# nygenome/lancet

Hardware: AMD Instinct MI355X
Metric: assembled windows/sec (whole node), 600bp windows, self-tuning k, synthetic T/N (higher is better)
Workload: dtype u64; 1 GPU; chr22-scan proxy: 32768 windows/GPU x 600 bp, stride 100, 30x tumor / 30x normal, 2x150 bp, k=11..101, active-region-off; windows_per_gpu=32768, reads_per_gpu=5895305, records_rank0_contig=22477, slots_in_flight=4080, batches_in_flight=2, windows_first_graph_in_lds=32768, graphs_built_ahead=2147, graphs_taken_from_pool=2037, windows_rerun_worst_case_tier=0

## Files before the change

lancet_amd/csrc/build_lds_impl.h:

```cpp
namespace BL_NS {

#if BL_OFFBITS > 16
typedef uint32_t bl_occ_t;
typedef uint32_t bl_off_t;
#else
typedef uint16_t bl_occ_t;
typedef uint16_t bl_off_t;
#endif
static constexpr uint32_t BL_OFFMASK = (1u << BL_OFFBITS) - 1u;
#if BL_WIDE
typedef uint32_t bl_on_t;
static constexpr uint32_t ON_ID = 0xFFFFFu, ON_OVL = 0x40000000u, ON_ORI = 0x80000000u, ON_ORISH = 31u;
#else
typedef uint16_t bl_on_t;
static constexpr uint32_t ON_ID = 0x1FFFu, ON_OVL = 0x4000u, ON_ORI = 0x8000u, ON_ORISH = 15u;
#endif
static_assert(BL_NCAP <= ON_ID + 1u && BL_SLOTS <= ON_ID + 1u && BL_NCAP < 65536u, "node ids / slots in a per-occurrence word");
static constexpr uint32_t LDS_BASES = BL_BASES, LDS_READS = BL_RMAX;
static_assert(BL_BASES < (1u << BL_OFFBITS) && BL_BASES / 16 + 4 < 65536, "offsets of the packed reads");

struct BlShared {
  uint32_t bases[BL_BASES / 16 + 4];
  uint32_t goodm[BL_BASES / 32 + 4];
  uint16_t rdo[BL_RMAX + 4];
// ... 5 lines not shown
  uint8_t prole[BL_RMAX + 4];
#if !BL_WIDE
  uint16_t idoff[BL_NCAP];
#endif
  alignas(8) uint16_t cidx[BL_NCAP];
  uint16_t t2c[BL_TCAP];
  alignas(16) uint32_t big[BL_BIG / 4];
  uint32_t wsum[BL_WG / 64 + 1];
  uint32_t scan_total;
  int w, R, reflen, K, hasN, mapped;
  uint32_t O, N, T, ncand, nsurv, nbw, ngw;
  uint32_t totalreadbp, n_kmers;
  int repE, repM;
  int why;
  uint32_t npairs, flagged, edges_total, refn;
  uint32_t g0, g1;
  uint32_t hint;
  uint32_t ndup;
  unsigned long long t_last, ph_acc[16]; int ph_cur;
};

struct BlScratch {
  LC_GLOBAL bl_on_t *occn;
  LC_GLOBAL uint32_t *idoff;
  LC_GLOBAL unsigned long long *tcc;
  LC_GLOBAL uint32_t *tfl;
  LC_GLOBAL uint32_t *c_id;
  LC_GLOBAL uint32_t *c_ti;
  LC_GLOBAL uint32_t *c_minqv;
  LC_GLOBAL uint32_t *s_ci;
  LC_GLOBAL uint32_t *s_edges;
  LC_GLOBAL bl_off_t *dupo;
  LC_GLOBAL uint32_t *ord;
  LC_GLOBAL uint32_t *pq;
};
static constexpr uint32_t BL_PQCAP = 16384u;
static constexpr uint32_t SCRATCH_BYTES = (((uint32_t)sizeof(bl_on_t) * BL_BASES + 64u + (BL_WIDE ? 4u * BL_NCAP + 64u : 64u) + 8u * BL_TCAP + 4u * BL_TCAP + 12u * PB_CCAP + 4u * PB_SCAP + 36u * PB_SCAP + (uint32_t)sizeof(bl_off_t) * BL_DUPCAP + 16u * PB_CMAX + 4u * 16384u + 768u) + 255u) & ~255u;
static constexpr int WG = BL_WG;
DEV void bl_scratch_carve(BlScratch *s, LC_GLOBAL uint8_t *base) {
  size_t o = 0;
  auto take = [&](size_t bytes) { LC_GLOBAL uint8_t *p = base + o; o = (o + bytes + 63) & ~(size_t)63; return p; };
  s->occn = (LC_GLOBAL bl_on_t *)take(sizeof(bl_on_t) * BL_BASES + 64u);
  s->idoff = (LC_GLOBAL uint32_t *)take(BL_WIDE ? 4u * BL_NCAP : 4u);
  s->tcc = (LC_GLOBAL unsigned long long *)take(8u * BL_TCAP);
  s->tfl = (LC_GLOBAL uint32_t *)take(4u * BL_TCAP);
  s->c_id = (LC_GLOBAL uint32_t *)take(4u * PB_CCAP);
  s->c_ti = (LC_GLOBAL uint32_t *)take(4u * PB_CCAP);
  s->c_minqv = (LC_GLOBAL uint32_t *)take(4u * PB_CCAP);
  s->s_ci = (LC_GLOBAL uint32_t *)take(4u * PB_SCAP);
  s->s_edges = (LC_GLOBAL uint32_t *)take(36u * PB_SCAP);
  s->dupo = (LC_GLOBAL bl_off_t *)take(sizeof(bl_off_t) * BL_DUPCAP);
  s->ord = (LC_GLOBAL uint32_t *)take(16u * PB_CMAX);
  s->pq = (LC_GLOBAL uint32_t *)take(4u * BL_PQCAP);
}

static_assert(sizeof(BlShared) <= BL_LDS_LIMIT, "LDS of the build kernel: 2 x 80 KB (512 lanes) or 1 x 160 KB (1024 lanes) per CU");
typedef LC_LDS BlShared BL_S;
#ifndef LANCET_WAVE_EMU
static __shared__ BlShared bl_shared;
template <class P> DEV unsigned long long dev_atomic_add64(P p, unsigned long long v) { return __hip_atomic_fetch_add(p, v, __ATOMIC_RELAXED, __HIP_MEMORY_SCOPE_WORKGROUP); }
template <class P> DEV unsigned long long dev_atomic_or64(P p, unsigned long long v) { return __hip_atomic_fetch_or(p, v, __ATOMIC_RELAXED, __HIP_MEMORY_SCOPE_WORKGROUP); }
#else
DEV unsigned long long dev_atomic_add64(unsigned long long *p, unsigned long long v) { unsigned long long o = *p; *p = o + v; return o; }
DEV unsigned long long dev_atomic_or64(unsigned long long *p, unsigned long long v) { unsigned long long o = *p; *p = o | v; return o; }
#endif

#define bl_bcast(p) wg_bcastu(p)

template <class T> DEV void bl_scan_t(LC_LDS T *a, int n, BL_S &S) {
  WG_SYNC();
#ifndef LANCET_WAVE_EMU
  const int t = (int)threadIdx.x, chunk = (n + BL_WG - 1) / BL_WG;
  int lo = t * chunk, hi = lo + chunk; if (lo > n) lo = n; if (hi > n) hi = n;
  uint32_t s = 0;
  for (int i = lo; i < hi; ++i) s += a[i];
  uint32_t inc = s; const int lane = t & 63;
  for (int d = 1; d < 64; d <<= 1) { const uint32_t x = (uint32_t)__shfl_up((int)inc, d, 64); if (lane >= d) inc += x; }
  if (lane == 63) S.wsum[t >> 6] = inc;
  __syncthreads();
  uint32_t woff = 0;
  for (int i = 0; i < (t >> 6); ++i) woff += S.wsum[i];
  uint32_t run = woff + inc - s;
  for (int i = lo; i < hi; ++i) { const uint32_t x = a[i]; a[i] = (T)run; run += x; }
  if (t == BL_WG - 1) S.scan_total = run;
  __syncthreads();
// ... 231 lines not shown
template <class F> DEV void bl_for_occ(BL_S &S, LC_GLOBAL const bl_on_t *occn, F body) {
  bl_for_chunk(S, occn, [&](const BlChunk &ch, const BlOccW &w) {
    for (int j = 0; j < ch.nv; ++j) body(ch.r, ch.p0 + j, ch.boff0 + (uint32_t)j, bl_occw_get(w, j));
  });
}
DEV void bl_chunk_bases(const LC_LDS uint32_t *bases, int c, unsigned long long &lo, unsigned long long &hi) {
  const uint32_t wd = (uint32_t)c >> 1;
  lo = (unsigned long long)bases[wd] | ((unsigned long long)bases[wd + 1] << 32); hi = (unsigned long long)bases[wd + 2];
  if (c & 1) { lo = (lo >> 16) | (hi << 48); hi >>= 16; }
}


#ifdef LANCET_PROF_A
#define BLPA(S, id) BLP(S, id)
#else
#define BLPA(S, id) ((void)0)
#endif
#ifdef LANCET_PROF_ORDER
#define BLPO(S, id) BLP(S, id)
#else
#define BLPO(S, id) ((void)0)
#endif
#define BLC_TO(e) ((uint32_t)(e) & 0x3FFu)
#define BLC_DIR(e) (((uint32_t)(e) >> 10) & 3u)
#define BLC_MAKE(to, dir) ((uint16_t)((to) | ((dir) << 10)))
DEVNI void bl_compress_first(LC_GLOBAL const lancet_params *P, LC_GLOBAL const EngineCaps *C, BL_S &S, BlScratch &X, LC_GLOBAL uint8_t *area, const int K_,
                             const uint32_t N_, const uint32_t nsurv_, const uint32_t ncand_, const int reflen_, const uint32_t ht_bc_, const uint32_t refmask_) {
  P = lc_sgpr(P); C = lc_sgpr(C); area = lc_sgpr(area);
  const uint32_t N = lc_sgpr(N_), nsurv = lc_sgpr(nsurv_), ncand = lc_sgpr(ncand_), ht_bc = lc_sgpr(ht_bc_); const int reflen = lc_sgpr(reflen_);
  const int K = lc_sgpr(K_); const uint32_t refmask = lc_sgpr(refmask_);
  LC_GLOBAL const PreLayout &PL = C->pl;
  LC_GLOBAL PreCmp *CH = (LC_GLOBAL PreCmp *)(area + PRE_OFF_CHDR);
  LC_GLOBAL const uint32_t *occ_ref = (LC_GLOBAL const uint32_t *)(area + PRE_OFF_OCCREF);
  LC_GLOBAL const unsigned long long *nhash = (LC_GLOBAL const unsigned long long *)(area + PRE_OFF_NHASH);
  LC_GLOBAL const unsigned long long *skey = (LC_GLOBAL const unsigned long long *)(area + PRE_OFF_SKEY);
  LC_GLOBAL const uint32_t *sidv = (LC_GLOBAL const uint32_t *)(area + PRE_OFF_SID);
  LC_GLOBAL NodeGr *pgr = (LC_GLOBAL NodeGr *)(area + PRE_OFF_PGR);
  LC_GLOBAL const uint16_t *qv = (LC_GLOBAL const uint16_t *)(area + PRE_OFF_QV);
  LC_GLOBAL uint32_t *clive = (LC_GLOBAL uint32_t *)(area + PRE_OFF_CLIVE);
  LC_GLOBAL uint32_t *cseq = (LC_GLOBAL uint32_t *)(area + PRE_OFF_CSEQ);
  const uint32_t Pn = nsurv + 2u, SRC = nsurv, SNK = nsurv + 1u;
  const bool recov = lc_sgpr((int)P->kmer_recovery) != 0;
  LC_LDS uint8_t *arena = (LC_LDS uint8_t *)&S.bases[0];
  LC_LDS uint16_t *pos2si = (LC_LDS uint16_t *)(arena + 70304);
  LC_LDS uint16_t *E = (LC_LDS uint16_t *)arena;
  LC_LDS uint8_t *NE = arena + 13376;
  LC_LDS uint8_t *FL = arena + 14272;
  LC_LDS uint16_t *SI2POS = (LC_LDS uint16_t *)(arena + 15168);
  LC_LDS uint32_t *LNK = (LC_LDS uint32_t *)(arena + 16896);
  LC_LDS unsigned long long *PT = (LC_LDS unsigned long long *)(arena + 23616);
  LC_LDS uint32_t *HS = (LC_LDS uint32_t *)(arena + 36992);
  LC_LDS uint32_t *AL = (LC_LDS uint32_t *)(arena + 40384);
  LC_LDS uint16_t *HEADOF = (LC_LDS uint16_t *)(arena + 43776);
  LC_LDS uint8_t *INFO = arena + 45504;
  LC_LDS uint16_t *HX = (LC_LDS uint16_t *)(arena + 46400);
  LC_LDS uint16_t *HL = (LC_LDS uint16_t *)(arena + 48128);
  LC_LDS uint32_t *HACC = (LC_LDS uint32_t *)(arena + 48640);
  LC_LDS uint16_t *NEWE = (LC_LDS uint16_t *)(arena + 52736);
  LC_LDS uint16_t *NPOS = (LC_LDS uint16_t *)(arena + 59392);
  LC_LDS unsigned long long *ORD = (LC_LDS unsigned long long *)(arena + 59392);
  LC_LDS unsigned long long *TCC = (LC_LDS unsigned long long *)(arena + 74400);
  LC_LDS uint16_t *CI = (LC_LDS uint16_t *)(arena + 67584);
  static_assert(74400 + 8 * PB_CMAX <= offsetof(BlShared, big) + BL_BIG && 8 * PB_CMAX <= 2 * 4096 && 67584 + 2 * PB_CMAX <= 70304, "compress arena (2)");
  static_assert(13376 >= (PB_CMAX + 2) * 16 && 14272 - 13376 >= PB_CMAX + 2 && 16896 - 15168 >= 2 * PB_CMAX && 23616 - 16896 >= 8 * (PB_CMAX + 2) &&
                36992 - 23616 >= 16 * (PB_CMAX + 2) && 40384 - 36992 >= 4 * (PB_CMAX + 3) && 45504 - 43776 >= 2 * (PB_CMAX + 2) && 48128 - 46400 >= 2 * (PB_CMAX + 2) &&
                52736 - 48640 >= 16 * PB_CHEADS && 59392 - 52736 >= 26 * PB_CHEADS && 59392 + 2 * 4096 <= 70304, "compress arena");
  WG_LANE0 { CH->done = 0; S.why = 0; S.flagged = 0; S.g0 = 0x7FFFFFFFu; S.g1 = 0; S.ndup = 0; S.wsum[0] = 0; S.wsum[1] = 0; }
// ... 686 lines not shown
        const uint32_t id = pre[wd >> 1] + ((wd & 1u) ? (uint32_t)dev_popc(bm[wd - 1u]) : 0u) + (uint32_t)dev_popc(bm[wd] & ((1u << (off & 31u)) - 1u));
        tab[i] = id;
#if BL_WIDE
        X.idoff[id] = off;
#else
        S.idoff[id] = (uint16_t)off;
#endif
      }
    }
    WG_SYNC();
  }
  const uint32_t N = bl_bcast(&S.N);
  BLP(S, 6);
  if (C->debug_stop == 106u) { WG_LANE0 { H->why = 99; } return; }
  bl_for_chunk(S, X.occn, [&](const BlChunk &ch, const BlOccW &w) {
    uint32_t old[8];
    BL_UNROLL for (int j = 0; j < 8; ++j) {
      const bool act = j < ch.nv;
      const uint32_t e = bl_occw_get(w, j);
      old[j] = dev_atomic_add(&tab[act ? (e & (nslots - 1)) : 0u], act ? (1u << 16) : 0u);
    }
    BlOccW o = {};
    BL_UNROLL for (int j = 0; j < 8; ++j) {
      if (BL_BASES > 65535u && j < ch.nv && (old[j] >> 16) >= 0xFFFEu) S.why = BLW_SIZE;
      bl_occw_set(o, j, j < ch.nv ? ((old[j] & 0xFFFFu) | (bl_occw_get(w, j) & ON_ORI)) : 0u);
    }
    bl_occw_store(X.occn, ch.boff0, o);
  });
  WG_SYNC();
  if (BL_BASES > 65535u) { if (bl_bcast(&S.why)) { WG_LANE0 { H->why = (uint32_t)S.why; } return; } }
  BLP(S, 7);
  if (C->debug_stop == 107u) { WG_LANE0 { H->why = 99; } return; }
  {
    LC_GLOBAL unsigned long long *nhash = (LC_GLOBAL unsigned long long *)(area + PRE_OFF_NHASH);
    LC_GLOBAL uint8_t *surv = (LC_GLOBAL uint8_t *)(area + PRE_OFF_SURV);
    WG_FULL_BEGIN(n, act, N)
      unsigned long long h;
#if BL_KW > 1
      if (NW > 1) {
        BlKm v, ck, alt; bool f; bl_kmer_x(S.bases, bl_idoff(S, X, (uint32_t)n), NW, K, v); bl_canon_x(v, NW, K, ck, alt, &f);
        h = bl_std_hash_km(ck, NW, K);
      } else
#endif
      { bool f; const unsigned long long ck = bl_canon(bl_kmer(S.bases, bl_idoff(S, X, (uint32_t)n), kmask), K, kmask, &f);
        h = std_hash_bytes([&](int j) -> int { return bl_acgt((int)((ck >> (2 * (K - 1 - j))) & 3ULL)); }, K); }
      if (act) { nhash[n] = h; surv[n] = 0; }
    WG_FULL_END
  }
  const double avgcov = ((double)S.totalreadbp) / ((double)reflen);
  int tmin = 1;
  while ((tmin <= P->low_cov_threshold) || ((double)tmin <= (P->min_cov_ratio * avgcov))) ++tmin;
  const uint32_t tthr = tmin < 2 ? (uint32_t)tmin : 2u;
  WG_FOR(i, nslots) { const uint32_t e = tab[i]; if (e != BL_EMPTY) S.cidx[e & 0xFFFFu] = (uint16_t)(e >> 16); }
  WG_SYNC();
  {
    const uint32_t nd = S.ndup < BL_DUPCAP ? S.ndup : BL_DUPCAP;
    const uint32_t cthr = (uint32_t)(avgcov / 4.0) > 4u ? (uint32_t)(avgcov / 4.0) : 4u;
    WG_FOR(i, nd) { if ((uint32_t)S.cidx[X.occn[X.dupo[i]] & ON_ID] < cthr) X.dupo[i] = (bl_off_t)~(bl_off_t)0; }
  }
  {
    LC_LDS uint32_t *fl = S.big;
    WG_FOR(n, N + 1) { fl[n] = (n < (int)N && S.cidx[n] >= tthr) ? 1u : 0u; }
    bl_scan32(fl, (int)N + 1, S);
    WG_LANE0 { S.T = S.scan_total; if (S.scan_total > BL_TCAP) S.why = BLW_TRACKED; }
    if (bl_bcast(&S.why)) { WG_LANE0 { H->why = (uint32_t)S.why; } return; }
    WG_FOR(n, N) { S.cidx[n] = (fl[n + 1] != fl[n]) ? (uint16_t)fl[n] : (uint16_t)0xFFFFu; }
    WG_SYNC();
// ... 563 lines not shown
      }
      WG_SYNC();
    }
  }
  BLP(S, 15);
  BL_TAIL_PRIO_SET(BL_TAIL_PRIO);
  WG_LANE0 { H->have_order = 0; }
  const bool wide_tab = BL_WIDE != 0 && N > 4096u;
  if ((N <= 4096u || (wide_tab && N <= BL_NCAP)) && nsurv > 0) {
    LC_LDS uint8_t *arena = (LC_LDS uint8_t *)&S.bases[0];
    LC_LDS uint32_t *first = (LC_LDS uint32_t *)arena;
    LC_LDS uint32_t *tmp = first + 5120;
    LC_LDS uint16_t *Qa = (LC_LDS uint16_t *)(tmp + 4104), *Qb = Qa + 4096, *bkt = Qb + 4096, *out = bkt + 4096;
    LC_LDS unsigned long long *nh = (LC_LDS unsigned long long *)(out + 4096);
    LC_LDS uint32_t *nx = (LC_LDS uint32_t *)(nh + 32), *bk = nx + 32;
    LC_LDS uint16_t *pos2si = (LC_LDS uint16_t *)(bk + 64);
    LC_LDS uint32_t *heads = (LC_LDS uint32_t *)(pos2si + PB_SCAP);
    static_assert(5120 * 4 + 4104 * 4 + 4 * 4096 * 2 + 32 * 8 + 32 * 4 + 64 * 4 + PB_SCAP * 2 + 128 * 4 <= offsetof(BlShared, big) + BL_BIG, "order arena");
    LC_LDS uint32_t *tmpP = tmp, *numP = first; LC_LDS uint16_t *nposP = (LC_LDS uint16_t *)first, *adjP = Qa;
#if BL_WIDE
    LC_LDS uint16_t *first16 = (LC_LDS uint16_t *)arena, *tmp16 = first16 + 20768, *bktw = nullptr;
    static_assert(BL_NCAP <= 14336 && BL_NCAP < 16384, "positions / run sizes in 16 bits, bucket counts up to 20 753");
    if (wide_tab) {
      Qa = tmp16 + 14352; Qb = Qa + 14336; bktw = Qb + 14336;
      nh = (LC_LDS unsigned long long *)(bktw + 14336); nx = (LC_LDS uint32_t *)(nh + 32); bk = nx + 32; pos2si = (LC_LDS uint16_t *)(bk + 64);
      tmpP = (LC_LDS uint32_t *)arena;
      numP = tmpP + 14352;
      nposP = bktw;
      adjP = (LC_LDS uint16_t *)(tmpP + 4104);
    }
    static_assert(2 * (20768 + 14352 + 3 * 14336) + 32 * 8 + 32 * 4 + 64 * 4 + PB_SCAP * 2 <= offsetof(BlShared, big) + BL_BIG && 4 * (14352 + PB_SCAP + 1) <= 2 * (20768 + 14352) &&
                  4 * 4104 + 2 * 8 * PB_SCAP <= 4 * 14337, "order arena of the large tables");
#endif
    LC_GLOBAL const unsigned long long *nhash = (LC_GLOBAL const unsigned long long *)(area + PRE_OFF_NHASH);
    const uint32_t SEQ = 13u;
    const uint32_t n0 = N < SEQ ? N : SEQ;
    WG_SYNC();
    WG_FOR(i, n0) { nh[i] = nhash[i]; }
    WG_LANE0 {
      uint32_t bc = 1, next_resize = 0, elt = 0, head = LC_NIL;
      bk[0] = LC_NIL;
      for (uint32_t n = 0; n < n0; ++n) {
        if (elt + 1 > next_resize) {
          unsigned long long mn = elt + 1;
          if (next_resize == 0 && mn < 11) mn = 11;
          if (mn >= bc) {
            unsigned long long want = mn + 1; if (want < 2ULL * bc) want = 2ULL * bc;
            const uint32_t nb = ht_next_prime((uint32_t)want);
            next_resize = nb;
            for (uint32_t i = 0; i < nb; ++i) bk[i] = LC_NIL;
            uint32_t pp = head; head = LC_NIL; uint32_t bbegin = 0;
            while (pp != LC_NIL) {
              const uint32_t nxt = nx[pp], b = ht_mod(nh[pp], nb);
              if (bk[b] == LC_NIL) { nx[pp] = head; head = pp; bk[b] = LC_BB; if (nx[pp] != LC_NIL) bk[bbegin] = pp; bbegin = b; }
              else { const uint32_t prev = bk[b]; if (prev == LC_BB) { nx[pp] = head; head = pp; } else { nx[pp] = nx[prev]; nx[prev] = pp; } }
              pp = nxt;
            }
            bc = nb;
          } else next_resize = bc;
        }
        const uint32_t b = ht_mod(nh[n], bc), prev = bk[b];
        if (prev != LC_NIL) { if (prev == LC_BB) { nx[n] = head; head = n; } else { nx[n] = nx[prev]; nx[prev] = n; } }
        else { nx[n] = head; head = n; if (nx[n] != LC_NIL) bk[ht_mod(nh[nx[n]], bc)] = n; bk[b] = LC_BB; }
        ++elt;
      }
      uint32_t m = 0;
      for (uint32_t pp = head; pp != LC_NIL; pp = nx[pp]) Qa[m++] = (uint16_t)pp;
// ... 136 lines not shown
        while (true) {
          a = uf_find(a); b = uf_find(b);
          if (a == b) break;
          const uint32_t hi = a > b ? a : b, lo = a > b ? b : a;
          if (dev_atomic_cas32(&parent[hi], hi, lo) == hi) break;
        }
      }
    }
    WG_SYNC();
    WG_FOR(u, nsurv) { const uint32_t r = uf_find((uint32_t)u); dev_atomic_min(&parent[u], r); }
    WG_SYNC();
#endif
    WG_FOR(u, nsurv) { if (touch[u] & 1u) dev_atomic_or(&touch[parent[u]], 2u); }
    WG_SYNC();
    LC_LDS uint32_t *num = numP;
    WG_FOR(u, nsurv + 1) { num[u] = (u < (int)nsurv && parent[u] == (uint32_t)u) ? 1u : 0u; }
    bl_scan32(num, (int)nsurv + 1, S);
    WG_LANE0 { S.nbw = S.scan_total; S.ngw = 0; S.flagged = 0; }
    WG_SYNC();
    WG_FOR(u, nsurv) { if (parent[u] == (uint32_t)u && (touch[u] & 2u)) { dev_atomic_add((LC_LDS uint32_t *)&S.ngw, 1u); if (num[u] < 32u) dev_atomic_or((LC_LDS uint32_t *)&S.flagged, 1u << num[u]); } }
    LC_GLOBAL NodeGr *pgr2 = (LC_GLOBAL NodeGr *)(area + PRE_OFF_PGR);
    WG_FOR(u, nsurv) { pgr2[pos2si[u]].comp = (int)(num[parent[u]] + 1u); }
    WG_LANE0 { H->have_order = 1; H->ht_bc = S.g0; H->ht_next_resize = S.g1; H->numcomp = S.nbw; H->refcomp = S.ngw; }
    WG_SYNC();
    BLPA(S, 15); BLPO(S, 15);
    {
      WG_SYNC();
      const uint32_t hbc = lc_sgpr((uint32_t)S.g0), hnr = lc_sgpr((uint32_t)S.g1), ncomp = lc_sgpr((uint32_t)S.nbw), refmask = lc_sgpr((uint32_t)S.flagged);
      WG_SYNC();
      if ((!rep || cmp_later) && (ncomp == 1u || (!rep && ncomp <= 32u)) && nsurv <= PB_CMAX && nsurv + 2u <= hnr && K <= 31 && !wide_tab && C->debug_stop != 140u && !P->lr_mode)
        bl_compress_first(P, C, S, X, area, K, N, nsurv, ncand, reflen, hbc, refmask);
    }
  }
  BL_TAIL_PRIO_SET(0);
  WG_LANE0 {
    H->K = K; H->refE = S.repE; H->refM = S.repM; H->N = S.N; H->O = S.O; H->totalreadbp = S.totalreadbp; H->n_kmers = S.n_kmers;
    H->ncand = S.ncand; H->nsurv = S.nsurv; H->edges_total = S.edges_total; H->refn = S.refn; H->why = 0; H->heavy = S.hint;
    H->big = BL_WG > 512 ? 1u : 0u;
    H->status = PB_BUILT;
  }
  WG_SYNC();
}

#ifndef BL_END_G
#define BL_END_G 512
#endif
DEV void build_kernel_body(LC_GLOBAL const lancet_params *P, LC_GLOBAL const DevBatch *B, LC_GLOBAL const EngineCaps *C, LC_GLOBAL uint8_t *pre,
                           LC_GLOBAL uint8_t *scratch, LC_GLOBAL uint32_t *queue, BL_S &S, int slot, LC_GLOBAL unsigned long long *phase = nullptr,
                           LC_GLOBAL uint8_t *pool = nullptr, uint32_t pool_cap = 0, int depth = 0, LC_GLOBAL uint32_t *biglist = nullptr, bool from_list = false,
                           bool wait_all = false, int cycle = 0) {
  LC_GLOBAL const PreLayout &PL = C->pl;
  LC_GLOBAL uint8_t *xbase = scratch + (size_t)slot * SCRATCH_BYTES;
  int done_here = 0;
  if (from_list && queue[4] == 0u) return;
  while (true) {
    WG_LANE0 { S.w = (int)dev_atomic_add(queue + (from_list ? 5 : 0), 1u); }
    int w = (int)bl_bcast(&S.w);
    if (from_list) { if ((uint32_t)w >= queue[4]) break; w = (int)biglist[w]; }
    else if (w >= B->n_windows) {
#ifndef LANCET_WAVE_EMU
      if (wait_all) { WG_LANE0 { while (ld_acq(queue + 7) < (uint32_t)B->n_windows) dev_sleep(); } WG_SYNC(); }
#endif
      break;
    }
#ifndef LANCET_WAVE_EMU
    if (threadIdx.x == 0) { if (phase) { for (int i = 0; i < 16; ++i) S.ph_acc[i] = 0; S.ph_cur = 0; S.t_last = wall_clock64(); } else S.ph_cur = -1; }
// ... 115 lines not shown
```

lancet_amd/csrc/kernels.h:

```cpp
#pragma once
#include "wave.h"
#include "layout.h"
#include "../../include/lancet_engine.h"

#ifndef LANCET_WG
#define LANCET_WG 64
#endif
#ifdef LANCET_FAT
#define LC_QLANES LC_FAT_LANES
#define LC_PF_G 6
#define LC_QSTAGE (3 * LC_FAT_LANES)
#else
#define LC_QLANES LANCET_WG
#define LC_QSTAGE LC_STAGE
#endif

enum {
  EV_PROCESS = 1, EV_REPEAT_REF, EV_NEAR_REF, EV_READS, EV_STATS, EV_MARKREF, EV_LOWCOV, EV_CLEANDEAD,
  EV_COMPRESS, EV_CC, EV_CCID, EV_CCEND, EV_TRIM, EV_AMBIG_SRC, EV_NOMATCH_SRC, EV_AMBIG_SNK, EV_NOMATCH_SNK,
  EV_CYCLE, EV_TIPS_ROUND, EV_TIPS_REMOVED, EV_LINKS, EV_LOOKREP, EV_MISSING, EV_SEARCH, EV_NEAR_QRY,
  EV_DFSLIMIT, EV_PATH, EV_TS, EV_PATH_END, EV_EKA_END, EV_FOUND, EV_END
};

struct WinShared {
// ... 4928 lines not shown
    if (rv >> 31) {
      for (int q = 0; q < 4; ++q) v[q] = W.gr[X].kc[q];
      for (int q = 0; q < 6; ++q) h[q] = W.khp[6 * (size_t)X + q];
    }
    if (i == 0) { for (int j = 0; j < K; ++j) { for (int q = 0; q < 4; ++q) W.refcov[4 * j + q] = v[q]; for (int q = 0; q < 6; ++q) W.refhp[6 * j + q] = h[q]; } }
    else { for (int q = 0; q < 4; ++q) W.refcov[4 * (i + K - 1) + q] = v[q]; for (int q = 0; q < 6; ++q) W.refhp[6 * (i + K - 1) + q] = h[q]; }
  }
  WG_LANE0 { uint32_t tcap = 1024; while (tcap < 2u * nsurv + 2u && tcap < LC_CTX(c).C->table_cap) tcap <<= 1; S.tmask = tcap - 1u; S.tfull = 0; }
  const uint32_t mask = wg_bcastu(&S.tmask);
  WG_FOR(i, mask + 1u) { lc_u4 z; z.x = 0; z.y = 0; z.z = LC_NIL; z.w = 0; *(lc_u4 *)(W.slots + 4 * (size_t)i) = z; }
  WG_SYNC_FENCE();
  WG_FOR(ci, ncand) {
    const uint32_t n = snode[ci];
    if (n == LC_NIL) continue;
    unsigned long long ck[LC_NWMAX];
    for (int w = 0; w < LC_NWMAX; ++w) ck[w] = w < NW ? skey[(size_t)ci * PL.kw + (uint32_t)w] : 0ULL;
    unsigned long long h = 0; uint32_t idx;
    if (NW == 1 && K <= 31) { h = ck[0] + 1ULL; idx = (uint32_t)mix64(h) & mask; }
    else {
      for (int w = 0; w < NW; ++w) h = mix64(h ^ (ck[w] + 0x9e3779b97f4a7c15ULL * (unsigned long long)(w + 1)));
      h &= ~(1ULL << 63);
      if (h == 0) h = 1;
      idx = (uint32_t)h & mask;
    }
    for (uint32_t probes = 0; probes <= mask; ++probes) {
      const unsigned long long old = dev_atomic_cas64(&SL_TAG(W, idx), 0ULL, h);
      if (old == 0ULL) { SL_NODE(W, idx) = n; if (!(NW == 1 && K <= 31)) for (int w = 0; w < NW; ++w) W.slot_key[(size_t)idx * LC_NWMAX + w] = ck[w]; break; }
      idx = (idx + 1) & mask;
    }
  }
  WG_SYNC_FENCE();
}

DEVNI bool load_prebuilt(Ctx &c, int k) {
  LC_WS &S = LC_SREF(c); LC_GLOBAL Work &W = *LC_CTX(c).W;
  LC_GLOBAL const uint8_t *pre = LC_CTX(c).OUT->pre;
  if (!pre) return false;
  LC_GLOBAL const PreLayout &PL = LC_PL(c);
  LC_GLOBAL const uint8_t *area = pre + (size_t)S.w * PRE_STRIDE;
  LC_GLOBAL const PreHdr *H = (LC_GLOBAL const PreHdr *)(area + PRE_OFF_HDR);
  for (int hop = 0; hop < 16 && H->status == PB_BUILT && H->K < k && H->next != 0u && LC_CTX(c).OUT->pre_pool; ++hop) {
    area = LC_CTX(c).OUT->pre_pool + (size_t)(H->next - 1u) * PRE_STRIDE;
    H = (LC_GLOBAL const PreHdr *)(area + PRE_OFF_HDR);
  }
  WG_LANE0 { S.tmp1 = (H->status == PB_BUILT && H->K == k && H->N <= LC_CTX(c).C->node_cap && (size_t)H->ncand * (size_t)k <= (size_t)LC_CTX(c).C->qv_cap &&
                       H->ncand <= LC_CTX(c).C->surv_cap && (size_t)H->ncand * (size_t)k <= (size_t)LC_CTX(c).C->seq_cap) ? 1 : 0;
             if (S.LR && !(H->lr == 1u && H->have_order == 1u && H->lr_total <= LC_CTX(c).C->occ_cap)) S.tmp1 = 0; }
  if (!wg_bcast(&S.tmp1)) return false;
  const uint32_t N = H->N, ncand = H->ncand, nsurv = H->nsurv;
  const int K = k;
  WG_LANE0 {
    if (S.n_builds > 0 && LC_CTX(c).OUT->n_ahead_used) dev_atomic_add(LC_CTX(c).OUT->n_ahead_used, 1u);
    S.N = N; S.N_last = N; S.O = H->O; S.totalreadbp = (int)H->totalreadbp; S.n_kmers += (unsigned long long)H->n_kmers; ++S.n_builds;
    if (N > S.max_nodes) S.max_nodes = N;
    S.sum_nodes += N;
    S.nspecial = 0; S.qv_top = ncand; S.seq_top = ncand * (uint32_t)K; S.tmask = 0; S.tfull = 0; S.prebuilt = 1;
    S.pre_edges = H->edges_total; S.pre_refn = H->refn;
    W.occ_base[S.R - 1] = 0;
    S.pre_order = H->have_order == 1u ? 1 : 0;
    if (S.pre_order) {
      S.M = nsurv; S.ht_bc = H->ht_bc; S.ht_elt = nsurv; S.ht_next_resize = H->ht_next_resize; S.ht_head = LC_NIL;
      S.numcomp = (int)H->numcomp; S.refcomp = (int)H->refcomp;
    }
  }
  const bool pre_order = H->have_order == 1u;
  LC_GLOBAL const unsigned long long *nhash = (LC_GLOBAL const unsigned long long *)(area + PRE_OFF_NHASH);
  LC_GLOBAL const uint8_t *surv = (LC_GLOBAL const uint8_t *)(area + PRE_OFF_SURV);
  LC_GLOBAL const uint32_t *snode = (LC_GLOBAL const uint32_t *)(area + PRE_OFF_SNODE), *sid = (LC_GLOBAL const uint32_t *)(area + PRE_OFF_SID);
  LC_GLOBAL const unsigned long long *skey = (LC_GLOBAL const unsigned long long *)(area + PRE_OFF_SKEY);
  LC_GLOBAL const uint32_t *occ_ref = (LC_GLOBAL const uint32_t *)(area + PRE_OFF_OCCREF);
  LC_GLOBAL const lc_v4 *pgr = (LC_GLOBAL const lc_v4 *)(area + PRE_OFF_PGR);
  LC_GLOBAL const lc_v4 *qsrc = (LC_GLOBAL const lc_v4 *)(area + PRE_OFF_QV);
  const uint32_t dummy = LC_CTX(c).C->node_cap + LC_CTX(c).C->special_cap;
  LC_GLOBAL const PreCmp *CH = (LC_GLOBAL const PreCmp *)(area + PRE_OFF_CHDR);
  WG_LANE0 { S.tmp1 = (S.seq_t5 != 0 || S.seq_len != S.reflen) ? 1 : 0; }
  const bool trimmed_before = wg_bcast(&S.tmp1) != 0;
  const int t5_before = wg_uniform(S.seq_t5), len_before = wg_uniform(S.seq_len);
  const bool cdone = pre_order && CH->done == 1u && LC_CTX(c).C->special_cap >= 2u && CH->m_live <= LC_CTX(c).C->node_cap &&
                     (size_t)ncand * (size_t)K + CH->seqn <= (size_t)LC_CTX(c).C->seq_cap;
  WG_LANE0 { S.cmp_done = cdone ? 1 : 0; }
  if (cdone) {
    const uint32_t mlive = CH->m_live, seqn = CH->seqn, ncap = LC_CTX(c).C->node_cap;
    LC_GLOBAL const uint32_t *clive = (LC_GLOBAL const uint32_t *)(area + PRE_OFF_CLIVE);
    LC_GLOBAL const uint32_t *cseq = (LC_GLOBAL const uint32_t *)(area + PRE_OFF_CSEQ);
    WG_LANE0 {
      const int so = CH->src_off, ko = CH->snk_off;
      S.M = mlive; S.ht_elt = mlive; S.nspecial = 2; S.source = ncap; S.sink = ncap + 1u;
      S.seq_t5 = so; S.seq_len = ko - so + K; S.trim5 = so & 0xFFFF; S.trim3 = (S.reflen - ko - K) & 0xFFFF;
      S.seq_top = ncand * (uint32_t)K + seqn; S.cmp_dead = CH->dead; S.cmp_edges0 = CH->edges0; S.cmp_nsurv = nsurv; S.cmp_edges_all = CH->edges_all; S.cmp_n1 = CH->n_c1; S.cmp_refmask = CH->refmask;
    }
    WG_FOR(si, nsurv) {
      const uint32_t n = sid[si];
      LC_GLOBAL lc_v4 *dst = (LC_GLOBAL lc_v4 *)&W.gr[n];
      lc_v4 a = pgr[8 * (size_t)si]; const lc_v4 z = pgr[8 * (size_t)si + 7];
      a.x |= NF_DEAD;
      dst[0] = a; dst[7] = z;
    }
    WG_SYNC();
    WG_FOR(i, mlive) {
      const uint32_t idx = clive[i];
      const bool sp = (idx & 0x80000000u) != 0;
      const uint32_t ri = sp ? nsurv + (idx & 0xFFu) : idx;
      const uint32_t id = sp ? ncap + (idx & 0xFFu) : sid[ri];
      W.order[i] = id;
      W.nhash[id] = sp ? CH->spec_hash[idx & 0xFFu] : nhash[id];
      lc_v4 r[8];
      for (int q = 0; q < 8; ++q) r[q] = pgr[8 * (size_t)ri + q];
      for (int q = 1; q < 4; ++q) {
        if (ED_TO(r[q].x) >= PB_SPECIAL) r[q].x = (r[q].x & 0xF0000000u) | (ncap + (ED_TO(r[q].x) - PB_SPECIAL));
        if (ED_TO(r[q].y) >= PB_SPECIAL) r[q].y = (r[q].y & 0xF0000000u) | (ncap + (ED_TO(r[q].y) - PB_SPECIAL));
        if (ED_TO(r[q].z) >= PB_SPECIAL) r[q].z = (r[q].z & 0xF0000000u) | (ncap + (ED_TO(r[q].z) - PB_SPECIAL));
        if (ED_TO(r[q].w) >= PB_SPECIAL) r[q].w = (r[q].w & 0xF0000000u) | (ncap + (ED_TO(r[q].w) - PB_SPECIAL));
      }
      LC_GLOBAL lc_v4 *dst = (LC_GLOBAL lc_v4 *)&W.gr[id];
      for (int q = 0; q < 8; ++q) dst[q] = r[q];
      const uint32_t nqv = r[7].x, slo = r[5].z, shi = r[5].w;
      if (!sp && nqv != LC_NIL && slo == nqv * (uint32_t)K && shi == slo + (uint32_t)K) {
        for (int t = 0; t < K; ++t) W.seq[slo + (uint32_t)t] = SD_MAKE(id, t, pre_key_base(skey, PL.kw, nqv, K, t));
      }
    }
    { const uint32_t base = ncand * (uint32_t)K; WG_FOR(i, seqn) { W.seq[base + (uint32_t)i] = cseq[i]; } }
    WG_LANE0 { S.seq_lazy = 0; }
    const uint32_t nch = CH->cov_heads;
    if (nch) {
      LC_GLOBAL const unsigned long long *cord = (LC_GLOBAL const unsigned long long *)(area + PRE_OFF_CORD);
      LC_GLOBAL const uint32_t *chl = (LC_GLOBAL const uint32_t *)(area + PRE_OFF_CHL);
      constexpr uint32_t LC_COV_CHUNK = 256u;
      static_assert(8u * LC_COV_CHUNK <= sizeof(S.lbytes), "merge operands staged in LDS");
      volatile LC_LDS unsigned long long *ops = (volatile LC_LDS unsigned long long *)&S.lbytes[0];
      const uint32_t nabs = CH->dead;
      WG_SYNC();
      for (uint32_t c0 = 0; c0 < nabs; c0 += LC_COV_CHUNK) {
        const uint32_t c1 = c0 + LC_COV_CHUNK < nabs ? c0 + LC_COV_CHUNK : nabs;
        WG_FOR(i, c1 - c0) { ops[i] = cord[c0 + (uint32_t)i]; }
        WG_SYNC();
        WG_FOR(x, 4 * nch) {
          const uint32_t hx = (uint32_t)x >> 2, q = (uint32_t)x & 3u;
          const uint32_t st = chl[3 * hx + 1], cnt = chl[3 * hx + 2];
          const uint32_t lo = st > c0 ? st : c0, hi = st + cnt < c1 ? st + cnt : c1;
          if (lo >= hi) continue;
          LC_GLOBAL NodeGr &G = W.gr[sid[chl[3 * hx]]];
          float nc = G.cov[q];
#ifndef LANCET_WAVE_EMU
          __builtin_amdgcn_s_setprio(3);
#endif
          float famer = (float)((int)(lo - st) + 1);
          for (uint32_t g = lo; g < hi; ++g) {
            const float bc = (float)(uint32_t)((ops[g - c0] >> (16 * q)) & 0xFFFFu);
            nc = ((nc * famer) + bc) / (famer + 1.0f);
            famer += 1.0f;
          }
#ifndef LANCET_WAVE_EMU
          __builtin_amdgcn_s_setprio(0);
#endif
          G.cov[q] = nc;
        }
        WG_SYNC();
      }
    }
  } else {
  if (pre_order) {
    LC_GLOBAL const uint32_t *ord = (LC_GLOBAL const uint32_t *)(area + PRE_OFF_ORDER);
    WG_FOR(i, nsurv) { const uint32_t n = ord[i]; W.order[i] = n; W.nhash[n] = nhash[n]; }
  } else { WG_FOR(n, N) { W.nhash[n] = nhash[n]; } }
  WG_FOR(l, LANCET_WG) {
    const int total = (int)(nsurv * 8u);
    for (int i0 = l; i0 < total; i0 += 4 * LANCET_WG) {
      lc_v4 v[4]; uint32_t dn[4];
      for (int u = 0; u < 4; ++u) { const int i = i0 + u * LANCET_WG; const int ic = i < total ? i : total - 1; v[u] = pgr[(size_t)ic]; dn[u] = sid[(uint32_t)ic >> 3]; }
      for (int u = 0; u < 4; ++u) { const int i = i0 + u * LANCET_WG; if (i < total) ((LC_GLOBAL lc_v4 *)&W.gr[dn[u]])[(uint32_t)i & 7u] = v[u]; }
    }
  }
  WG_LANE0 { S.seq_lazy = 1; S.lz_area = (unsigned long long)(uintptr_t)area; S.lz_skey = (unsigned long long)(uintptr_t)skey; S.lz_kw = PL.kw; }
  (void)snode; (void)skey;
  }
  WG_FOR(i, (N + 3) / 4) { ((LC_GLOBAL uint32_t *)W.survb)[i] = ((LC_GLOBAL const uint32_t *)surv)[i]; }
  WG_LANE0 { W.qv = (LC_GLOBAL uint16_t *)(area + PRE_OFF_QV); }
  (void)qsrc;
  const int nrefk = S.reflen - K > 0 ? S.reflen - K + 1 : 0;
  WG_FOR(i, nrefk) { const uint32_t e = occ_ref[i]; W.occ[i] = (e & PB_GONE) ? (dummy | (e & 0x80000000u)) : e; }
  WG_FOR(i, S.reflen * 2) { ((LC_GLOBAL uint32_t *)W.refcov)[i] = ((LC_GLOBAL const uint32_t *)(area + PRE_OFF_REFCOV))[i]; }
  WG_LANE0 { W.gr[dummy].flags = 0; }
  if (trimmed_before) {
    const int t5 = t5_before, L = len_before;
    WG_FOR(i, (N + 31u) / 32u) { W.bitmap[i] = 0; }
    WG_SYNC();
    WG_FOR(i, L - K > 0 ? L - K : 0) {
      const int p = t5 + i;
      if (p < nrefk) { const uint32_t n = occ_ref[p] & 0x3FFFFFFFu; dev_atomic_or(&W.bitmap[n >> 5], 1u << (n & 31u)); }
    }
    WG_SYNC();
    WG_LANE0 { S.tmp1 = 0; }
    WG_FOR(si, nsurv) {
      const uint32_t n = sid[si]; const uint32_t f = W.gr[n].flags;
      const bool in = ((ld2(&W.bitmap[n >> 5]) >> (n & 31u)) & 1u) != 0;
      W.gr[n].flags = in ? (f | NF_INMER) : (f & ~(uint32_t)NF_INMER);
      if (in) S.tmp1 = 1;
    }
    WG_SYNC();
    WG_LANE0 { if (S.cmp_done) S.refcomp = S.tmp1 ? 1 : 0; }
    WG_FOR(i, S.reflen - K > 0 ? S.reflen - K : 0) {
      const uint32_t n = occ_ref[i] & 0x3FFFFFFFu;
      if (!((ld2(&W.bitmap[n >> 5]) >> (n & 31u)) & 1u)) {
        if (i == 0) { for (int j = 0; j < K; ++j) for (int q = 0; q < 4; ++q) W.refcov[4 * j + q] = 0; }
        else { for (int q = 0; q < 4; ++q) W.refcov[4 * (i + K - 1) + q] = 0; }
      }
    }
    if (LC_CTX(c).C->evt_cap) {
      WG_LANE0 { uint32_t cnt = 0; for (uint32_t i = 0; i < (N + 31u) / 32u; ++i) cnt += (uint32_t)dev_popc(ld2(&W.bitmap[i])); S.pre_refn = cnt; }
    }
  }
  WG_SYNC();
  if (wg_uniform(S.LR)) load_prebuilt_lr(c, area);
  return true;
// ... 359 lines not shown
```

Measured before the change: 877,600 windows/s.

## Stage node hashes in scratch and vectorize prebuilt-graph copy loops with ILP

The build kernel now writes and reads node hashes in a per-workgroup scratch buffer and copies them back to the prebuilt area at the end, touching only live or surviving nodes when an order exists. Separately, load_prebuilt's copies of graph records, sequence words, survival bytes, reference occurrences and coverage are rewritten as 16-byte vector loads with several loads in flight per lane. The goal is fewer scalar global transactions and better latency hiding in the copy loops. In exchange, scratch grows by 8 bytes per node capacity, an extra copy-back pass is added, and the vector casts assume 16-byte-aligned source and destination buffers.

```diff
diff --git a/lancet_amd/csrc/build_lds_impl.h b/lancet_amd/csrc/build_lds_impl.h
--- a/lancet_amd/csrc/build_lds_impl.h
+++ b/lancet_amd/csrc/build_lds_impl.h
@@ -61,10 +61,11 @@
   LC_GLOBAL uint32_t *s_edges;
   LC_GLOBAL bl_off_t *dupo;
   LC_GLOBAL uint32_t *ord;
+  LC_GLOBAL unsigned long long *nhash;
   LC_GLOBAL uint32_t *pq;
 };
 static constexpr uint32_t BL_PQCAP = 16384u;
-static constexpr uint32_t SCRATCH_BYTES = (((uint32_t)sizeof(bl_on_t) * BL_BASES + 64u + (BL_WIDE ? 4u * BL_NCAP + 64u : 64u) + 8u * BL_TCAP + 4u * BL_TCAP + 12u * PB_CCAP + 4u * PB_SCAP + 36u * PB_SCAP + (uint32_t)sizeof(bl_off_t) * BL_DUPCAP + 16u * PB_CMAX + 4u * 16384u + 768u) + 255u) & ~255u;
+static constexpr uint32_t SCRATCH_BYTES = (((uint32_t)sizeof(bl_on_t) * BL_BASES + 64u + (BL_WIDE ? 4u * BL_NCAP + 64u : 64u) + 8u * BL_TCAP + 4u * BL_TCAP + 12u * PB_CCAP + 4u * PB_SCAP + 36u * PB_SCAP + (uint32_t)sizeof(bl_off_t) * BL_DUPCAP + 16u * PB_CMAX + 8u * BL_NCAP + 4u * 16384u + 832u) + 255u) & ~255u;
 static constexpr int WG = BL_WG;
 DEV void bl_scratch_carve(BlScratch *s, LC_GLOBAL uint8_t *base) {
   size_t o = 0;
@@ -80,6 +81,7 @@
   s->s_edges = (LC_GLOBAL uint32_t *)take(36u * PB_SCAP);
   s->dupo = (LC_GLOBAL bl_off_t *)take(sizeof(bl_off_t) * BL_DUPCAP);
   s->ord = (LC_GLOBAL uint32_t *)take(16u * PB_CMAX);
+  s->nhash = (LC_GLOBAL unsigned long long *)take(8u * BL_NCAP);
   s->pq = (LC_GLOBAL uint32_t *)take(4u * BL_PQCAP);
 }
 
@@ -377,7 +379,7 @@
   LC_GLOBAL const PreLayout &PL = C->pl;
   LC_GLOBAL PreCmp *CH = (LC_GLOBAL PreCmp *)(area + PRE_OFF_CHDR);
   LC_GLOBAL const uint32_t *occ_ref = (LC_GLOBAL const uint32_t *)(area + PRE_OFF_OCCREF);
-  LC_GLOBAL const unsigned long long *nhash = (LC_GLOBAL const unsigned long long *)(area + PRE_OFF_NHASH);
+  LC_GLOBAL const unsigned long long *nhash = X.nhash;
   LC_GLOBAL const unsigned long long *skey = (LC_GLOBAL const unsigned long long *)(area + PRE_OFF_SKEY);
   LC_GLOBAL const uint32_t *sidv = (LC_GLOBAL const uint32_t *)(area + PRE_OFF_SID);
   LC_GLOBAL NodeGr *pgr = (LC_GLOBAL NodeGr *)(area + PRE_OFF_PGR);
@@ -1130,7 +1132,7 @@
   BLP(S, 7);
   if (C->debug_stop == 107u) { WG_LANE0 { H->why = 99; } return; }
   {
-    LC_GLOBAL unsigned long long *nhash = (LC_GLOBAL unsigned long long *)(area + PRE_OFF_NHASH);
+    LC_GLOBAL unsigned long long *nhash = X.nhash;
     LC_GLOBAL uint8_t *surv = (LC_GLOBAL uint8_t *)(area + PRE_OFF_SURV);
     WG_FULL_BEGIN(n, act, N)
       unsigned long long h;
@@ -1760,7 +1762,7 @@
     static_assert(2 * (20768 + 14352 + 3 * 14336) + 32 * 8 + 32 * 4 + 64 * 4 + PB_SCAP * 2 <= offsetof(BlShared, big) + BL_BIG && 4 * (14352 + PB_SCAP + 1) <= 2 * (20768 + 14352) &&
                   4 * 4104 + 2 * 8 * PB_SCAP <= 4 * 14337, "order arena of the large tables");
 #endif
-    LC_GLOBAL const unsigned long long *nhash = (LC_GLOBAL const unsigned long long *)(area + PRE_OFF_NHASH);
+    LC_GLOBAL const unsigned long long *nhash = X.nhash;
     const uint32_t SEQ = 13u;
     const uint32_t n0 = N < SEQ ? N : SEQ;
     WG_SYNC();
@@ -1963,6 +1965,23 @@
         bl_compress_first(P, C, S, X, area, K, N, nsurv, ncand, reflen, hbc, refmask);
     }
   }
+  {
+    LC_GLOBAL const PreCmp *CHd = (LC_GLOBAL const PreCmp *)(area + PRE_OFF_CHDR);
+    WG_LANE0 { S.g0 = H->have_order;
+               const bool take = CHd->done == 1u && C->special_cap >= 2u && CHd->m_live <= C->node_cap && CHd->m_live <= S.N && (size_t)S.ncand * (size_t)K + CHd->seqn <= (size_t)C->seq_cap;
+               S.g1 = take ? CHd->m_live : 0u; }
+    const uint32_t ordered = lc_sgpr((uint32_t)S.g0), mlive = lc_sgpr((uint32_t)S.g1);
+    LC_GLOBAL unsigned long long *nh_out = (LC_GLOBAL unsigned long long *)(area + PRE_OFF_NHASH);
+    LC_GLOBAL const uint32_t *sid_o = (LC_GLOBAL const uint32_t *)(area + PRE_OFF_SID);
+    if (ordered && mlive) {
+      LC_GLOBAL const uint32_t *clive_o = (LC_GLOBAL const uint32_t *)(area + PRE_OFF_CLIVE);
+      WG_FOR(i, mlive) { const uint32_t idx = clive_o[i]; if (!(idx & 0x80000000u)) { const uint32_t n = sid_o[idx]; nh_out[n] = X.nhash[n]; } }
+    } else if (ordered) {
+      WG_FOR(si, S.nsurv) { const uint32_t n = sid_o[si]; nh_out[n] = X.nhash[n]; }
+    } else {
+      WG_FOR(n, S.N) { nh_out[n] = X.nhash[n]; }
+    }
+  }
   BL_TAIL_PRIO_SET(0);
   WG_LANE0 {
     H->K = K; H->refE = S.repE; H->refM = S.repM; H->N = S.N; H->O = S.O; H->totalreadbp = S.totalreadbp; H->n_kmers = S.n_kmers;
diff --git a/lancet_amd/csrc/kernels.h b/lancet_amd/csrc/kernels.h
--- a/lancet_amd/csrc/kernels.h
+++ b/lancet_amd/csrc/kernels.h
@@ -4984,6 +4984,22 @@
   WG_SYNC_FENCE();
 }
 
+template <class F> DEV void wg_copy_words(LC_GLOBAL uint32_t *dst, LC_GLOBAL const uint32_t *src, uint32_t nw, F f) {
+  const int nv = (int)(nw >> 2);
+  LC_GLOBAL const lc_v4 *s4 = (LC_GLOBAL const lc_v4 *)src; LC_GLOBAL lc_v4 *d4 = (LC_GLOBAL lc_v4 *)dst;
+  WG_FOR_ILP(i0, nv) {
+    lc_v4 v[LC_ILP];
+    for (int u = 0; u < LC_ILP; ++u) { const int i = i0 + u * LC_ILP_STRIDE; v[u] = s4[i < nv ? i : nv - 1]; }
+    for (int u = 0; u < LC_ILP; ++u) {
+      const int i = i0 + u * LC_ILP_STRIDE;
+      if (i >= nv) continue;
+      lc_v4 t = v[u]; t.x = f(t.x); t.y = f(t.y); t.z = f(t.z); t.w = f(t.w);
+      d4[i] = t;
+    }
+  }
+  WG_FOR(t, nw & 3u) { dst[4u * (uint32_t)nv + (uint32_t)t] = f(src[4u * (uint32_t)nv + (uint32_t)t]); }
+}
+
 DEVNI bool load_prebuilt(Ctx &c, int k) {
   LC_WS &S = LC_SREF(c); LC_GLOBAL Work &W = *LC_CTX(c).W;
   LC_GLOBAL const uint8_t *pre = LC_CTX(c).OUT->pre;
@@ -5041,12 +5057,18 @@
       S.seq_t5 = so; S.seq_len = ko - so + K; S.trim5 = so & 0xFFFF; S.trim3 = (S.reflen - ko - K) & 0xFFFF;
       S.seq_top = ncand * (uint32_t)K + seqn; S.cmp_dead = CH->dead; S.cmp_edges0 = CH->edges0; S.cmp_nsurv = nsurv; S.cmp_edges_all = CH->edges_all; S.cmp_n1 = CH->n_c1; S.cmp_refmask = CH->refmask;
     }
-    WG_FOR(si, nsurv) {
-      const uint32_t n = sid[si];
-      LC_GLOBAL lc_v4 *dst = (LC_GLOBAL lc_v4 *)&W.gr[n];
-      lc_v4 a = pgr[8 * (size_t)si]; const lc_v4 z = pgr[8 * (size_t)si + 7];
-      a.x |= NF_DEAD;
-      dst[0] = a; dst[7] = z;
+    WG_FOR_ILP(s0, nsurv) {
+      uint32_t n[LC_ILP]; lc_v4 a[LC_ILP], z[LC_ILP];
+      for (int u = 0; u < LC_ILP; ++u) {
+        const int si = s0 + u * LC_ILP_STRIDE; const size_t sc = (size_t)(si < (int)nsurv ? si : (int)nsurv - 1);
+        n[u] = sid[sc]; a[u] = pgr[8 * sc]; z[u] = pgr[8 * sc + 7];
+      }
+      for (int u = 0; u < LC_ILP; ++u) {
+        if (s0 + u * LC_ILP_STRIDE >= (int)nsurv) continue;
+        LC_GLOBAL lc_v4 *dst = (LC_GLOBAL lc_v4 *)&W.gr[n[u]];
+        a[u].x |= NF_DEAD;
+        dst[0] = a[u]; dst[7] = z[u];
+      }
     }
     WG_SYNC();
     WG_FOR(i, mlive) {
@@ -5071,7 +5093,21 @@
         for (int t = 0; t < K; ++t) W.seq[slo + (uint32_t)t] = SD_MAKE(id, t, pre_key_base(skey, PL.kw, nqv, K, t));
       }
     }
-    { const uint32_t base = ncand * (uint32_t)K; WG_FOR(i, seqn) { W.seq[base + (uint32_t)i] = cseq[i]; } }
+    {
+      const uint32_t base = ncand * (uint32_t)K; const int nv = (int)(seqn >> 2);
+      LC_GLOBAL const lc_v4 *c4 = (LC_GLOBAL const lc_v4 *)cseq;
+      WG_FOR_ILP(i0, nv) {
+        lc_v4 v[LC_ILP];
+        for (int u = 0; u < LC_ILP; ++u) { const int i = i0 + u * LC_ILP_STRIDE; v[u] = c4[i < nv ? i : nv - 1]; }
+        for (int u = 0; u < LC_ILP; ++u) {
+          const int i = i0 + u * LC_ILP_STRIDE;
+          if (i >= nv) continue;
+          LC_GLOBAL uint32_t *d = W.seq + base + 4u * (uint32_t)i;
+          d[0] = v[u].x; d[1] = v[u].y; d[2] = v[u].z; d[3] = v[u].w;
+        }
+      }
+      WG_FOR(t, seqn & 3u) { W.seq[base + 4u * (uint32_t)nv + (uint32_t)t] = cseq[4u * (uint32_t)nv + (uint32_t)t]; }
+    }
     WG_LANE0 { S.seq_lazy = 0; }
     const uint32_t nch = CH->cov_heads;
     if (nch) {
@@ -5126,12 +5162,12 @@
   WG_LANE0 { S.seq_lazy = 1; S.lz_area = (unsigned long long)(uintptr_t)area; S.lz_skey = (unsigned long long)(uintptr_t)skey; S.lz_kw = PL.kw; }
   (void)snode; (void)skey;
   }
-  WG_FOR(i, (N + 3) / 4) { ((LC_GLOBAL uint32_t *)W.survb)[i] = ((LC_GLOBAL const uint32_t *)surv)[i]; }
+  wg_copy_words((LC_GLOBAL uint32_t *)W.survb, (LC_GLOBAL const uint32_t *)surv, (N + 3) / 4, [](uint32_t x) { return x; });
   WG_LANE0 { W.qv = (LC_GLOBAL uint16_t *)(area + PRE_OFF_QV); }
   (void)qsrc;
   const int nrefk = S.reflen - K > 0 ? S.reflen - K + 1 : 0;
-  WG_FOR(i, nrefk) { const uint32_t e = occ_ref[i]; W.occ[i] = (e & PB_GONE) ? (dummy | (e & 0x80000000u)) : e; }
-  WG_FOR(i, S.reflen * 2) { ((LC_GLOBAL uint32_t *)W.refcov)[i] = ((LC_GLOBAL const uint32_t *)(area + PRE_OFF_REFCOV))[i]; }
+  wg_copy_words(W.occ, occ_ref, (uint32_t)nrefk, [dummy](uint32_t e) { return (e & PB_GONE) ? (dummy | (e & 0x80000000u)) : e; });
+  wg_copy_words((LC_GLOBAL uint32_t *)W.refcov, (LC_GLOBAL const uint32_t *)(area + PRE_OFF_REFCOV), (uint32_t)(wg_uniform(S.reflen) * 2), [](uint32_t x) { return x; });
   WG_LANE0 { W.gr[dummy].flags = 0; }
   if (trimmed_before) {
     const int t5 = t5_before, L = len_before;
```

Result: no change. 884,900 windows/s, median of 6 (+0.8%).
